# handasontam/PERT-GNN-KDD23

Measured on AMD Instinct MI355X. Metric: training graphs/sec (whole node), higher is better.
Workload: dtype bf16; 1 GPU; model=PERT-GNN 8L/256H, global_batch=1024, vocab=realistic, interfaces=2041, entry_unions=266, graph_mode=full, parallelism=dp1

## Files before the change

csrc/bindings.cpp:

```cpp
#include <hip/hip_runtime.h>
#include <torch/extension.h>

#include <climits>
#include <cstdlib>
#include <memory>
#include <optional>
#include <string>
#include <vector>

#include <c10/cuda/CUDAStream.h>

#include "hip/attn_bn.h"
#include "hip/gemm_dispatch.h"

namespace {

#define CHECK_IN(t)                                                      \
  TORCH_CHECK((t).is_cuda(), #t " must be on GPU");                      \
  TORCH_CHECK((t).is_contiguous(), #t " must be contiguous")

inline hipStream_t cur_stream() {
  return (hipStream_t)c10::cuda::getCurrentCUDAStream().stream();
}

// ... 147 lines not shown
void launch_gemm_f32_nt(const float*, const float*, const float*, float*, int,
                        int, int, bool, hipStream_t);
void launch_gemm_f32_nn(const float*, const float*, const float*, float*, int,
                        int, int, bool, hipStream_t);
void launch_gemm_f32_tn(const float*, const float*, float*, float*, int, int,
                        int, hipStream_t);
void launch_colsum(const float*, float*, long, int, hipStream_t);
void launch_gemm_bf16_nt(const float*, const float*, const float*, float*,
                         int, int, int, bool, hipStream_t);
void launch_gemm_bf16_nn(const float*, const float*, const float*, float*,
                         int, int, int, bool, hipStream_t);
void launch_gemm_bf16_tn(const float*, const float*, float*, float*, int, int,
                         int, hipStream_t);
void launch_gemm_fp16_nt(const float*, const float*, const float*, float*,
                         int, int, int, bool, hipStream_t);
void launch_gemm_fp16_nn(const float*, const float*, const float*, float*,
                         int, int, int, bool, hipStream_t);
void launch_gemm_fp16_tn(const float*, const float*, float*, float*, int, int,
                         int, hipStream_t);
void launch_embed_grouped_scatter(const float*, const int*, const int*, float*,
                                  float*, long, int, int, int, int, int,
                                  hipStream_t);
void launch_embed_grouped_scatter_bal(const void*, int, const int*,
                                      const int*, const int*, const int*,
                                      const int*, const int*, float*, float*,
                                      float*, int, int, int, int, int, int,
                                      hipStream_t);
void launch_rows_sum_lists(const void*, int, const int*, const int*, void*, int,
                           int, int, int, hipStream_t);
void launch_rows_sum_lists_wide(const void*, int, int, const int*, const int*,
                                float*, int, int, int, int, int, hipStream_t);
void launch_embed_fold_gemm(const float*, const float*, float*, int, int, int,
                            int, int, bool, hipStream_t);
void launch_vocab_scatter(const float*, const long*, long, float*, long, int,
                          int, int, int, hipStream_t);
void launch_vocab_scatter_dual(const float*, const long*, int, float*, float*,
                               long, int, int, int, hipStream_t);
void launch_edge_attn_fused_fwd(const float*, const float*, const float*,
                                const long*, int, const int*, const int*,
                                float*, float*, int, int, int, hipStream_t);
void launch_edge_attn_fused_bwd(const float*, const float*, const float*,
                                const float*, const long*, int, const float*,
                                const int*, const int*, const int*,
                                const int*, const int*, float*, float*,
                                float*, int, int, long, int, hipStream_t);
void launch_edge_attn_fused_fwd16(const void*, const void*, const void*,
                                  int, const long*, int, const int*,
                                  const int*, void*, int, float*, int, int,
                                  int, hipStream_t);
void launch_edge_attn_fused_bwd16(const void*, int, const void*,
                                  const void*, const void*, int, const long*,
                                  int, const float*, const int*, const int*,
                                  const int*, const int*, const int*, void*,
                                  void*, float*, int, int, long, int,
                                  hipStream_t, const AttnBnBwd* = nullptr,
                                  const AttnPoolBwd* = nullptr);
void launch_bn_bwd_partials_affine16(const void*, const void*,
                                     const unsigned char*, const float*,
                                     const float*, long, int, float*, float,
                                     float*, float*, float*, hipStream_t,
                                     bool acc = false);
void launch_edge_attn_fused_infer(const float*, const float*, const float*,
                                  const long*, int, const int*, const int*,
                                  const float*, const float*, int, float*,
                                  int, int, int, hipStream_t);
void launch_edge_attn_fused_infer16(const void*, const void*, const void*,
                                    int, const long*, int, const int*,
                                    const int*, const float*, const float*,
                                    int, void*, int, int, int, int,
                                    hipStream_t);
void launch_vocab_scatter_dual16(const void*, const long*, int, float*,
                                 float*, long, int, int, int, hipStream_t);
void launch_gemm_bf16_nt_o16(const float*, const float*, const float*, void*,
                             int, int, int, hipStream_t);
void launch_gemm_a16_glds_nt(const void*, const void*, const float*, void*,
                             int, int, int, int, bool, hipStream_t);
void launch_convert_w16(const float*, void*, long, hipStream_t);
void launch_convert_w16_both(const float*, void*, void*, int, int,
                             hipStream_t);
void launch_gemm_a16_glds_tn(const void*, const void*, float*, float*, int,
                             int, int, hipStream_t, bool acc = false,
                             int tile = 0);
int glds_tn_tile_for(int m, int n, int k2, int tile);
void set_glds_tn_tile(int tile);
void launch_transpose_convert_w16(const float*, void*, int, int, hipStream_t);
void launch_gemm_skinny_nn(const void*, const float*, float*, int, int, int,
                           hipStream_t);
void launch_gemm_bf16_nn_a16(const void*, const float*, float*, int, int, int,
                             hipStream_t);
void launch_gemm_bf16_tn_a16(const void*, const float*, float*, float*, int,
                             int, int, hipStream_t, bool acc = false);
int ptables_max_groups();
void launch_ptables_fwd(int, const float* const*, const float* const*,
                        void* const*, const int*, int, int, hipStream_t);
void launch_ptables_dgrad(const void* const*, const float* const*, const int*,
                          float* const*, const int*, int, int, const bool*,
                          hipStream_t);
bool launch_ptables_wgrad(int, const void* const*, const float* const*,
                          float* const*, const int*, int, bool, hipStream_t,
                          const bool* sink = nullptr);
std::vector<torch::Tensor> collate_native(
    std::vector<torch::Tensor>, std::vector<torch::Tensor>,
    std::vector<torch::Tensor>, std::vector<torch::Tensor>,
    std::vector<torch::Tensor>, std::vector<torch::Tensor>,
    std::vector<torch::Tensor>, std::vector<torch::Tensor>,
    std::vector<torch::Tensor>, bool);


std::vector<torch::Tensor> edge_attn_fwd(torch::Tensor q, torch::Tensor k,
                                         torch::Tensor v, torch::Tensor e,
                                         torch::Tensor row_ptr,
                                         torch::Tensor csr_src,
                                         torch::Tensor skip) {
  CHECK_IN(q); CHECK_IN(k); CHECK_IN(v); CHECK_IN(e);
  CHECK_IN(row_ptr); CHECK_IN(csr_src);
  const int n = q.size(0);
  const int h = q.size(1);
  TORCH_CHECK(h <= 512, "H must be <= 512");
  auto out = torch::empty_like(q);
  auto alpha = torch::empty({e.size(0)}, q.options());
  const float* skip_p = nullptr;
  if (skip.defined() && skip.numel() > 0) {
    CHECK_IN(skip);
    skip_p = skip.data_ptr<float>();
  }
  launch_edge_attn_fwd(q.data_ptr<float>(), k.data_ptr<float>(),
                       v.data_ptr<float>(), e.data_ptr<float>(),
                       row_ptr.data_ptr<int>(), csr_src.data_ptr<int>(),
                       skip_p, out.data_ptr<float>(), alpha.data_ptr<float>(),
                       n, h, cur_stream());
  return {out, alpha};
}

std::vector<torch::Tensor> edge_attn_bwd(
    torch::Tensor g, torch::Tensor q, torch::Tensor k, torch::Tensor v,
    torch::Tensor e, torch::Tensor alpha, torch::Tensor row_ptr,
    torch::Tensor csr_src, torch::Tensor col_ptr, torch::Tensor csc_dst,
    torch::Tensor csc_eid) {
  CHECK_IN(g); CHECK_IN(q); CHECK_IN(alpha);
  const int n = q.size(0);
  const int h = q.size(1);
  const long ne = e.size(0);
  auto dq = torch::empty_like(q);
  auto dk = torch::empty_like(k);
  auto dv = torch::empty_like(v);
  auto de = torch::empty_like(e);
  auto dek = torch::empty_like(e);
  auto dev = torch::empty_like(e);
  launch_edge_attn_bwd(g.data_ptr<float>(), q.data_ptr<float>(),
                       k.data_ptr<float>(), v.data_ptr<float>(),
                       e.data_ptr<float>(), alpha.data_ptr<float>(),
                       row_ptr.data_ptr<int>(), csr_src.data_ptr<int>(),
                       col_ptr.data_ptr<int>(), csc_eid.data_ptr<int>(),
                       dq.data_ptr<float>(), dk.data_ptr<float>(),
                       dv.data_ptr<float>(), de.data_ptr<float>(),
                       dek.data_ptr<float>(), dev.data_ptr<float>(), n, h, ne,
                       cur_stream());
  return {dq, dk, dv, de};
}

torch::Tensor seg_pool_fwd(torch::Tensor x, torch::Tensor probs,
                           torch::Tensor nn, torch::Tensor batch_ptr,
                           int64_t num_graphs) {
  CHECK_IN(x); CHECK_IN(probs); CHECK_IN(nn); CHECK_IN(batch_ptr);
  const int h = x.size(1);
  const long n = x.size(0);
// ... 1185 lines not shown
    torch::Tensor csc_dst, torch::Tensor csc_eid, int64_t heads = 1) {
  CHECK_IN(gout); CHECK_IN(probs); CHECK_IN(nn); CHECK_IN(batch);
  CHECK_IN(qkvs); CHECK_IN(alpha);
  const int n = qkvs.size(0);
  const int h = qkvs.size(1) / 4;
  const long ne = ea.size(0);
  TORCH_CHECK(h == 256 || h == 512, "edge_attn_pool_bwd16 covers H = 256, 512");
  TORCH_CHECK(qkvs.scalar_type() == torch::kBFloat16,
              "edge_attn_pool_bwd16 takes bf16 qkvs");
  TORCH_CHECK(gout.scalar_type() == torch::kFloat32 && gout.dim() == 2 &&
                  gout.size(1) == h,
              "gout must be fp32 [graphs, h]");
  TORCH_CHECK(probs.scalar_type() == torch::kFloat32 &&
                  nn.scalar_type() == torch::kFloat32 &&
                  batch.scalar_type() == torch::kInt64 &&
                  probs.numel() == n && nn.numel() == n && batch.numel() == n,
              "probs/nn (fp32) and batch (int64) must have one entry per node");
  TORCH_CHECK(heads >= 1 && heads <= h && h % heads == 0,
              "heads must divide H (H=", h, ", heads=", heads, ")");
  TORCH_CHECK(alpha.scalar_type() == torch::kFloat32 &&
                  alpha.numel() == ne * heads,
              "alpha must be the fp32 [E, heads] tensor of the forward");
  TORCH_CHECK(pifc.scalar_type() == prpc.scalar_type(),
              "P tables must share a dtype");
  AttnPoolBwd pool{};
  pool.gout = gout.data_ptr<float>();
  pool.probs = probs.data_ptr<float>();
  pool.nn = nn.data_ptr<float>();
  pool.batch = batch.data_ptr<long>();
  auto fopt = qkvs.options().dtype(torch::kFloat32);
  auto dqkvs = torch::empty_like(qkvs);
  auto de = torch::empty({ne, h}, qkvs.options());
  auto dal = torch::empty({ne * heads}, fopt);
  const int p16 = pifc.scalar_type() == torch::kBFloat16 ? 1 : 0;
  launch_edge_attn_fused_bwd16(
      nullptr, 0, qkvs.data_ptr(), pifc.data_ptr(), prpc.data_ptr(), p16,
      ea.data_ptr<long>(), (int)ea.size(1), alpha.data_ptr<float>(),
      row_ptr.data_ptr<int>(), csr_src.data_ptr<int>(),
      col_ptr.data_ptr<int>(), csc_dst.data_ptr<int>(),
      csc_eid.data_ptr<int>(), dqkvs.data_ptr(), de.data_ptr(),
      dal.data_ptr<float>(), n, h, ne, (int)heads, cur_stream(), nullptr,
      &pool);
  return {dqkvs, de};
}

torch::Tensor seg_pool_fwd16(torch::Tensor x, torch::Tensor probs,
                             torch::Tensor nn, torch::Tensor batch_ptr,
                             int64_t num_graphs) {
  CHECK_IN(x); CHECK_IN(probs); CHECK_IN(nn); CHECK_IN(batch_ptr);
  const int h = x.size(1);
  const long n = x.size(0);
  long p = 8192 / std::max<int64_t>(num_graphs, 1);
  const long per_g = (n + std::max<int64_t>(num_graphs, 1) - 1) /
                     std::max<int64_t>(num_graphs, 1);
  p = std::min<long>(std::max<long>(std::min(p, per_g), 1), 64);
  auto fopt = x.options().dtype(torch::kFloat32);
  auto partial = torch::empty({num_graphs * p, h}, fopt);
  auto out = torch::empty({num_graphs, h}, fopt);
  launch_seg_pool_fwd16(x.data_ptr(), probs.data_ptr<float>(),
                        nn.data_ptr<float>(), batch_ptr.data_ptr<int>(),
                        partial.data_ptr<float>(), out.data_ptr<float>(),
                        (int)num_graphs, (int)p, h, cur_stream());
  return out;
}

torch::Tensor seg_pool_bwd16(torch::Tensor gout, torch::Tensor probs,
                             torch::Tensor nn, torch::Tensor batch) {
  CHECK_IN(gout); CHECK_IN(batch);
  const long n = batch.size(0);
  const int h = gout.size(1);
  auto dx = torch::empty({n, h}, gout.options().dtype(torch::kBFloat16));
  launch_seg_pool_bwd16(gout.data_ptr<float>(), probs.data_ptr<float>(),
                        nn.data_ptr<float>(), batch.data_ptr<long>(),
                        dx.data_ptr(), n, h, cur_stream());
  return dx;
}

using gemm_dispatch::dgrad_glds_ok;

static std::vector<torch::Tensor> linear_fwd_a16o16_impl(torch::Tensor x,
                                                         torch::Tensor w,
                                                         torch::Tensor b,
                                                         bool fp16c,
                                                         bool want_wt) {
  CHECK_IN(x); CHECK_IN(w);
  const int m = x.size(0);
  const int k = x.size(1);
  const int n = w.size(0);
  auto y = torch::empty({m, n}, x.options());
  auto wt16 = torch::empty({0}, x.options());
  if (m == 0) return {y, wt16};
  const float* bias = nullptr;
  if (b.defined() && b.numel() > 0) bias = b.data_ptr<float>();
  if (fp16c) {
    launch_gemm_fp16_nt_a16o16(x.data_ptr(), w.data_ptr<float>(), bias,
                               y.data_ptr(), m, n, k, cur_stream());
    return {y, wt16};
  }
  if (gemm_dispatch::fwd_glds_ok(m, n, k)) {
    auto w16 = torch::empty({n, k}, x.options());
    if (want_wt && dgrad_glds_ok(m, n, k)) {
      wt16 = torch::empty({k, n}, x.options());
      launch_convert_w16_both(w.data_ptr<float>(), w16.data_ptr(),
                              wt16.data_ptr(), n, k, cur_stream());
    } else {
      launch_convert_w16(w.data_ptr<float>(), w16.data_ptr(), (long)n * k,
                         cur_stream());
    }
    launch_gemm_a16_glds_nt(x.data_ptr(), w16.data_ptr(), bias, y.data_ptr(),
                            1, m, n, k, false, cur_stream());
    return {y, wt16};
  }
  launch_gemm_bf16_nt_a16o16(x.data_ptr(), w.data_ptr<float>(), bias,
                             y.data_ptr(), m, n, k, cur_stream());
  return {y, wt16};
}

std::vector<torch::Tensor> convert_w16_both(torch::Tensor w) {
  CHECK_IN(w);
  TORCH_CHECK(w.scalar_type() == torch::kFloat32 && w.dim() == 2,
              "w must be fp32 [n, k]");
  const int n = w.size(0);
  const int k = w.size(1);
  auto opt = w.options().dtype(torch::kBFloat16);
  auto w16 = torch::empty({n, k}, opt);
  auto wt16 = torch::empty({k, n}, opt);
  launch_convert_w16_both(w.data_ptr<float>(), w16.data_ptr(),
                          wt16.data_ptr(), n, k, cur_stream());
  return {w16, wt16};
}

torch::Tensor linear_fwd_a16o16(torch::Tensor x, torch::Tensor w,
                                torch::Tensor b, bool fp16c = false) {
  return linear_fwd_a16o16_impl(x, w, b, fp16c, false)[0];
}

std::vector<torch::Tensor> linear_fwd_a16o16_wt(torch::Tensor x,
                                                torch::Tensor w,
                                                torch::Tensor b,
                                                bool fp16c = false) {
  return linear_fwd_a16o16_impl(x, w, b, fp16c, true);
}

torch::Tensor linear_dgrad16_o16(torch::Tensor g, torch::Tensor w,
                                 bool fp16c = false,
                                 c10::optional<torch::Tensor> wt16_in =
                                     c10::nullopt) {
  CHECK_IN(g); CHECK_IN(w);
  const int m = g.size(0);
  const int n = w.size(0);
  const int k = w.size(1);
  auto dx = torch::empty({m, k}, g.options());
  if (m == 0) return dx;
  if (fp16c) {
    launch_gemm_fp16_nn_a16o16(g.data_ptr(), w.data_ptr<float>(),
                               dx.data_ptr(), m, n, k, cur_stream());
    return dx;
  }
  if (dgrad_glds_ok(m, n, k)) {
    torch::Tensor wt16;
    if (wt16_in.has_value() && wt16_in->defined() && wt16_in->numel() > 0) {
      wt16 = *wt16_in;
      CHECK_IN(wt16);
      TORCH_CHECK(wt16.scalar_type() == torch::kBFloat16 && wt16.dim() == 2 &&
                      wt16.size(0) == k && wt16.size(1) == n,
                  "wt16 must be the bf16 [k, n] image of w");
    } else {
      wt16 = torch::empty({k, n}, g.options());
      launch_transpose_convert_w16(w.data_ptr<float>(), wt16.data_ptr(), n, k,
                                   cur_stream());
    }
    launch_gemm_a16_glds_nt(g.data_ptr(), wt16.data_ptr(), nullptr,
                            dx.data_ptr(), 1, m, k, n, false,
                            cur_stream());
    return dx;
  }
  launch_gemm_bf16_nn_a16o16(g.data_ptr(), w.data_ptr<float>(),
                             dx.data_ptr(), m, n, k, cur_stream());
  return dx;
}

std::vector<torch::Tensor> linear_wgrad16_b16(torch::Tensor g, torch::Tensor x,
                                              bool has_bias,
                                              bool fp16c = false,
                                              OptTensor dw_sink = std::nullopt,
                                              OptTensor db_sink = std::nullopt,
                                              int64_t tile = 0) {
  CHECK_IN(g); CHECK_IN(x);
  const int m = x.size(0);
  const int k = x.size(1);
  const int n = g.size(1);
  const char* det = getenv("PERTGNN_DETERMINISTIC");
  const bool glds = gemm_dispatch::wgrad_glds_ok(m, n, k, det && det[0] == '1');
  TORCH_CHECK(tile == 0 ||
                  (glds && !fp16c && glds_tn_tile_for(m, n, k, (int)tile) > 0),
              "linear_wgrad16_b16: tile ", tile, " cannot run [", m, ", ", n,
              "]^T x [", m, ", ", k, "] (needs bf16 compute, m >= 512, n "
              "and k multiples of the tile, not deterministic)");
  auto fopt = x.options().dtype(torch::kFloat32);
  float* dw_ptr = grad_sink(dw_sink, x, {n, k}, "linear_wgrad16_b16");
  float* db_ptr = grad_sink(db_sink, x, {n}, "linear_wgrad16_b16");
  const bool acc = dw_ptr != nullptr;
  TORCH_CHECK((db_ptr != nullptr) == (acc && has_bias),
              "linear_wgrad16_b16: a db sink comes with a dw sink and a bias");
  torch::Tensor dw = torch::empty({0}, fopt), db = torch::empty({0}, fopt);
  if (m == 0) {
    if (acc) return {dw, db};
    return {torch::zeros({n, k}, fopt), torch::zeros({has_bias ? n : 0}, fopt)};
  }
  if (!acc) {
    const long nk = (long)n * k;
    auto buf = torch::empty({nk + (has_bias ? n : 0)}, fopt);
    dw = buf.narrow(0, 0, nk).view({n, k});
    dw_ptr = dw.data_ptr<float>();
    if (has_bias) {
      db = buf.narrow(0, nk, n);
      db_ptr = db.data_ptr<float>();
    }
  }
  if (fp16c) {
    launch_gemm_fp16_tn_a16b16(g.data_ptr(), x.data_ptr(), dw_ptr, db_ptr, m,
                               n, k, cur_stream(), acc);
    return {dw, db};
  }
  if (glds) {
    launch_gemm_a16_glds_tn(g.data_ptr(), x.data_ptr(), dw_ptr, db_ptr, m, n,
                            k, cur_stream(), acc, (int)tile);
    return {dw, db};
  }
  launch_gemm_bf16_tn_a16b16(g.data_ptr(), x.data_ptr(), dw_ptr, db_ptr, m, n,
                             k, cur_stream(), acc);
  return {dw, db};
}

std::string linear_path(const std::string& op, int64_t m64, int64_t n64,
                        int64_t k64, const std::string& io, int64_t prec,
                        bool deterministic) {
  namespace gd = gemm_dispatch;
  TORCH_CHECK(m64 >= 0 && n64 > 0 && k64 > 0 && m64 <= INT_MAX &&
                  n64 <= INT_MAX && k64 <= INT_MAX,
              "linear_path: bad shape");
  const int m = (int)m64, n = (int)n64, k = (int)k64;
  const int iop = op == "fwd" ? 0 : op == "dgrad" ? 1 : op == "wgrad" ? 2 : -1;
  TORCH_CHECK(iop >= 0, "linear_path: op must be fwd, dgrad or wgrad");
  const bool f32io = io == "f32", o16 = io == "o16", a16 = io == "a16";
  TORCH_CHECK(f32io || o16 || a16, "linear_path: io must be f32, o16 or a16");
  TORCH_CHECK(f32io ? (prec >= 0 && prec <= 2)
                    : o16 ? prec == 1 : (prec == 1 || prec == 2),
              "linear_path: no binding with this io and prec");
  if (m == 0) return "none";
  const std::string fp16 = prec == 2 ? "_fp16" : "";
  const std::string fam = prec == 0 ? "f32" : "reg";
  const auto tile = [](bool big) { return big ? "128" : "64"; };
  if (iop == 0) {
    if (a16 && prec == 1 && gd::fwd_glds_ok(m, n, k))
      return gd::glds_nt_wide(m, n, k) ? "glds_nt_128x256" : "glds_nt_128x128";
    return fam + "_nt_" + tile(gd::tile128(m, n)) + fp16;
  }
  if (iop == 1) {
    if (a16 && prec == 1 && gd::dgrad_glds_ok(m, n, k))
      return gd::glds_nt_wide(m, k, n) ? "glds_nt_128x256" : "glds_nt_128x128";
    if (o16 && gd::dgrad_skinny(m)) return "skinny_nn";
    return fam + "_nn_" + tile(gd::tile128(m, k)) + fp16;
  }
  if (a16 && prec == 1 && gd::wgrad_glds_ok(m, n, k, deterministic))
    return "glds_tn/s=" +
           std::to_string(gd::glds_tn_slices(
               m, gd::glds_tn_tiles(gd::glds_tn_tile(m, n, k), n, k)));
  return fam + "_tn_" + tile(gd::tn_tile128(n, k)) + fp16 + "/s=" +
         std::to_string(gd::tn_slices(m, gd::tn_tiles(n, k),
                                      prec == 0 ? 32 : 64, deterministic));
}

std::string wgrad_tile(int64_t m, int64_t n, int64_t k, bool deterministic) {
  TORCH_CHECK(m >= 0 && n > 0 && k > 0 && m <= INT_MAX && n <= INT_MAX &&
                  k <= INT_MAX, "wgrad_tile: bad shape");
  if (!gemm_dispatch::wgrad_glds_ok((int)m, (int)n, (int)k, deterministic))
    return "none";
  return gemm_dispatch::tn_tile_name(
      glds_tn_tile_for((int)m, (int)n, (int)k, gemm_dispatch::TN_AUTO));
}

void set_wgrad_tile(int64_t tile) {
  TORCH_CHECK(tile >= 0 && tile <= gemm_dispatch::TN_256x256,
              "set_wgrad_tile: tile must be 0 (auto), 1, 2 or 3");
  set_glds_tn_tile((int)tile);
}

std::vector<std::string> linear_path_labels() {
  std::vector<std::string> out;
  const auto add = [&](const char* io, int prec, const char* op,
                       const std::string& label) {
    out.push_back(std::string(io) + "|" + std::to_string(prec) + "|" + op +
                  "|" + label);
  };
  const auto reg = [&](const char* io, int prec) {
    const std::string fam = prec == 0 ? "f32" : "reg";
    const std::string fp16 = prec == 2 ? "_fp16" : "";
    for (const char* t : {"64", "128"}) {
      add(io, prec, "fwd", fam + "_nt_" + t + fp16);
      add(io, prec, "dgrad", fam + "_nn_" + t + fp16);
      for (const char* s : {"/s=1", "/s>1"})
        add(io, prec, "wgrad", fam + "_tn_" + t + fp16 + s);
    }
  };
  for (int prec = 0; prec <= 2; ++prec) reg("f32", prec);
  reg("o16", 1);
  add("o16", 1, "dgrad", "skinny_nn");
  reg("a16", 1);
  reg("a16", 2);
  for (const char* op : {"fwd", "dgrad"})
    for (const char* l : {"glds_nt_128x128", "glds_nt_128x256"})
      add("a16", 1, op, l);
  for (const char* s : {"/s=1", "/s>1"})
    add("a16", 1, "wgrad", std::string("glds_tn") + s);
  return out;
}


namespace {

int ptables_check(const torch::Tensor& ifc_table,
                  const torch::Tensor& rpc_table,
                  const std::vector<torch::Tensor>& we_ifc,
                  const std::vector<torch::Tensor>& we_rpc) {
  CHECK_IN(ifc_table); CHECK_IN(rpc_table);
  TORCH_CHECK(ifc_table.dim() == 2 && rpc_table.dim() == 2,
              "ptables: tables must be 2-D");
  TORCH_CHECK(ifc_table.scalar_type() == torch::kFloat32 &&
                  rpc_table.scalar_type() == torch::kFloat32,
              "ptables: tables must be float32");
  const int64_t h = ifc_table.size(1);
  TORCH_CHECK(h > 0 && rpc_table.size(1) == h,
              "ptables: tables must share a non-empty hidden size");
  TORCH_CHECK(!we_ifc.empty() && we_ifc.size() == we_rpc.size(),
              "ptables: need one we_ifc and one we_rpc per layer, got ",
              we_ifc.size(), " and ", we_rpc.size());
  for (const auto* list : {&we_ifc, &we_rpc})
    for (const auto& w : *list) {
      TORCH_CHECK(w.is_cuda() && w.device() == ifc_table.device(),
                  "ptables: weight must be on the tables' GPU");
      TORCH_CHECK(w.is_contiguous(), "ptables: weight must be contiguous");
      TORCH_CHECK(w.scalar_type() == torch::kFloat32,
                  "ptables: weight must be float32");
      TORCH_CHECK(w.dim() == 2 && w.size(0) == h && w.size(1) == h,
                  "ptables: weight must be [", h, ", ", h, "]");
    }
  TORCH_CHECK(ifc_table.size(0) < (1 << 30) && rpc_table.size(0) < (1 << 30) &&
                  h < (1 << 15),
              "ptables: table too large");
  return (int)h;
}

}

std::vector<torch::Tensor> ptables_fwd(torch::Tensor ifc_table,
                                       torch::Tensor rpc_table,
                                       std::vector<torch::Tensor> we_ifc,
                                       std::vector<torch::Tensor> we_rpc) {
  const int h = ptables_check(ifc_table, rpc_table, we_ifc, we_rpc);
  const int layers = (int)we_ifc.size();
  auto opt = ifc_table.options().dtype(torch::kBFloat16);
  std::vector<torch::Tensor> out;
  std::vector<const float*> a, w;
  std::vector<void*> c;
  std::vector<int> m;
  for (int t = 0; t < 2; ++t) {
    const auto& table = t == 0 ? ifc_table : rpc_table;
    const auto& ws = t == 0 ? we_ifc : we_rpc;
// ... 164 lines not shown
          py::arg("relu"), py::arg("keep_inv") = 1.0,
          py::arg("dgamma_sink") = py::none(),
          py::arg("dbeta_sink") = py::none());
  mod.def("vocab_scatter", &vocab_scatter);
  mod.def("collate_native", &collate_native,
          py::call_guard<py::gil_scoped_release>());
  mod.def("edge_attn_fused_fwd", &edge_attn_fused_fwd, py::arg("qkvs"),
          py::arg("pifc"), py::arg("prpc"), py::arg("edge_attr"),
          py::arg("row_ptr"), py::arg("csr_src"), py::arg("out16"),
          py::arg("heads") = 1);
  mod.def("edge_attn_fused_bwd", &edge_attn_fused_bwd, py::arg("g"),
          py::arg("qkvs"), py::arg("pifc"), py::arg("prpc"),
          py::arg("edge_attr"), py::arg("alpha"), py::arg("row_ptr"),
          py::arg("csr_src"), py::arg("col_ptr"), py::arg("csc_dst"),
          py::arg("csc_eid"), py::arg("heads") = 1);
  mod.def("edge_attn_fused_infer", &edge_attn_fused_infer, py::arg("qkvs"),
          py::arg("pifc"), py::arg("prpc"), py::arg("edge_attr"),
          py::arg("row_ptr"), py::arg("csr_src"), py::arg("bn_scale"),
          py::arg("bn_shift"), py::arg("relu"), py::arg("out16"),
          py::arg("heads") = 1);
  mod.def("embed_grouped_scatter", &embed_grouped_scatter);
  mod.def("linear_fwd", &linear_fwd);
  mod.def("linear_fwd_bf16", &linear_fwd_bf16);
  mod.def("linear_fwd_fp16", &linear_fwd_fp16);
  mod.def("linear_bwd_fp16", &linear_bwd_fp16);
  mod.def("linear_bwd_bf16", &linear_bwd_bf16);
  mod.def("gemm_nt_bf16", &gemm_nt_bf16);
  mod.def("gemm_nn_bf16", &gemm_nn_bf16);
  mod.def("gemm_tn_bf16", &gemm_tn_bf16);
  mod.def("linear_bwd", &linear_bwd);
  mod.def("gemm_nt", &gemm_nt);
  mod.def("gemm_nn", &gemm_nn);
  mod.def("gemm_tn", &gemm_tn);
  mod.def("edge_attn_fwd", &edge_attn_fwd);
  mod.def("edge_attn_bwd", &edge_attn_bwd);
  mod.def("seg_pool_fwd", &seg_pool_fwd);
  mod.def("seg_pool_bwd", &seg_pool_bwd);
  mod.def("embed_node_fwd", &embed_node_fwd, py::arg("x_raw"), py::arg("idx"), py::arg("table"), py::arg("out16") = false, py::arg("pad_to") = 0);
  mod.def("embed_edge_fwd", &embed_edge_fwd);
  mod.def("gather_rows", &gather_rows);
  mod.def("bn_relu_fwd16", &bn_relu_fwd16, py::arg("x"), py::arg("gamma"),
          py::arg("beta"), py::arg("running_mean"), py::arg("running_var"),
          py::arg("momentum"), py::arg("eps"), py::arg("training"),
          py::arg("relu"), py::arg("dropout_p") = 0.0,
          py::arg("seed") = torch::Tensor());
  mod.def("bn_relu_bwd16", &bn_relu_bwd16, py::arg("g"), py::arg("x"),
          py::arg("gamma"), py::arg("mean"), py::arg("invstd"), py::arg("y"),
          py::arg("relu"), py::arg("keep_inv") = 1.0,
          py::arg("dgamma_sink") = py::none(),
          py::arg("dbeta_sink") = py::none());
  mod.def("bn_finalize_apply16", &bn_finalize_apply16, py::arg("x"),
          py::arg("partials"), py::arg("gamma"), py::arg("beta"),
          py::arg("running_mean"), py::arg("running_var"), py::arg("momentum"),
          py::arg("eps"), py::arg("training"), py::arg("relu"),
          py::arg("dropout_p") = 0.0, py::arg("seed") = torch::Tensor());
  mod.def("bn_bwd_partials16", &bn_bwd_partials16, py::arg("g"), py::arg("x"),
          py::arg("y"), py::arg("mean"), py::arg("invstd"), py::arg("relu"),
          py::arg("keep_inv") = 1.0);
  mod.def("bn_bwd_apply16", &bn_bwd_apply16, py::arg("g"), py::arg("x"),
          py::arg("y"), py::arg("mean"), py::arg("invstd"), py::arg("gamma"),
          py::arg("partials_global"), py::arg("partials_local"),
          py::arg("relu"), py::arg("keep_inv") = 1.0,
          py::arg("dgamma_sink") = py::none(),
          py::arg("dbeta_sink") = py::none());
  mod.def("edge_attn_bn_bwd16", &edge_attn_bn_bwd16, py::arg("g"),
          py::arg("x"), py::arg("mask"), py::arg("gamma"), py::arg("mean"),
          py::arg("invstd"), py::arg("keep_inv"), py::arg("qkvs"),
          py::arg("pifc"), py::arg("prpc"), py::arg("edge_attr"),
          py::arg("alpha"), py::arg("row_ptr"), py::arg("csr_src"),
          py::arg("col_ptr"), py::arg("csc_dst"), py::arg("csc_eid"),
          py::arg("heads") = 1, py::arg("partials_global") = py::none(),
          py::arg("partials_local") = py::none(),
          py::arg("dgamma_sink") = py::none(),
          py::arg("dbeta_sink") = py::none());
  mod.def("edge_attn_pool_bwd16", &edge_attn_pool_bwd16, py::arg("gout"),
          py::arg("probs"), py::arg("nn"), py::arg("batch"), py::arg("qkvs"),
          py::arg("pifc"), py::arg("prpc"), py::arg("edge_attr"),
          py::arg("alpha"), py::arg("row_ptr"), py::arg("csr_src"),
          py::arg("col_ptr"), py::arg("csc_dst"), py::arg("csc_eid"),
          py::arg("heads") = 1);
  mod.def("seg_pool_fwd16", &seg_pool_fwd16);
  mod.def("seg_pool_bwd16", &seg_pool_bwd16);
  mod.def("linear_fwd_a16o16", &linear_fwd_a16o16, py::arg("x"), py::arg("w"),
          py::arg("b"), py::arg("fp16c") = false);
  mod.def("convert_w16_both", &convert_w16_both, py::arg("w"));
  mod.def("linear_fwd_a16o16_wt", &linear_fwd_a16o16_wt, py::arg("x"),
          py::arg("w"), py::arg("b"), py::arg("fp16c") = false);
  mod.def("linear_dgrad16_o16", &linear_dgrad16_o16, py::arg("g"),
          py::arg("w"), py::arg("fp16c") = false,
          py::arg("wt16") = py::none());
  mod.def("linear_wgrad16_b16", &linear_wgrad16_b16, py::arg("g"),
          py::arg("x"), py::arg("has_bias"), py::arg("fp16c") = false,
          py::arg("dw_sink") = py::none(), py::arg("db_sink") = py::none(),
          py::arg("tile") = 0);
  mod.def("wgrad_tile", &wgrad_tile, py::arg("m"), py::arg("n"), py::arg("k"),
          py::arg("deterministic") = false);
  mod.def("set_wgrad_tile", &set_wgrad_tile, py::arg("tile"));
  mod.def("linear_path", &linear_path, py::arg("op"), py::arg("m"),
          py::arg("n"), py::arg("k"), py::arg("io"), py::arg("prec"),
          py::arg("deterministic") = false);
  mod.def("linear_path_labels", &linear_path_labels);
  mod.def("bn_relu_fwd", &bn_relu_fwd, py::arg("x"), py::arg("gamma"),
          py::arg("beta"), py::arg("running_mean"), py::arg("running_var"),
          py::arg("momentum"), py::arg("eps"), py::arg("training"),
          py::arg("relu"), py::arg("dropout_p") = 0.0,
          py::arg("seed") = torch::Tensor());
  mod.def("bn_relu_bwd", &bn_relu_bwd, py::arg("g"), py::arg("x"),
          py::arg("gamma"), py::arg("mean"), py::arg("invstd"), py::arg("y"),
          py::arg("relu"), py::arg("keep_inv") = 1.0,
          py::arg("dgamma_sink") = py::none(),
          py::arg("dbeta_sink") = py::none());
  mod.def("quantile_loss_fwd", &quantile_loss_fwd);
  mod.def("quantile_loss_bwd", &quantile_loss_bwd);
  mod.def("eval_metrics", &eval_metrics);
  mod.def("adam_step_dynamic", &adam_step_dynamic);
  mod.def("adam_step", &adam_step, py::arg("p"), py::arg("g"), py::arg("m"),
          py::arg("v"), py::arg("state"), py::arg("lr"), py::arg("b1"),
          py::arg("b2"), py::arg("eps"), py::arg("gscale") = 1.0);
}
```

csrc/hip/gemm_bf16.hip:

```cpp

#include "common.h"
#include "gemm_dispatch.h"

static inline bool pertgnn_deterministic() {
  const char* e = getenv("PERTGNN_DETERMINISTIC");
  return e && e[0] == '1';
}
#include <cstdlib>

#define BGEMM_PAD 8
#define BGEMM_THREADS 256

typedef __attribute__((ext_vector_type(4))) float f32x4;
typedef __attribute__((ext_vector_type(8))) __bf16 bf16x8;
typedef __attribute__((ext_vector_type(4))) __bf16 bf16x4;
typedef __attribute__((ext_vector_type(8))) _Float16 f16x8;
typedef __attribute__((ext_vector_type(4))) _Float16 f16x4;

template <typename T16> struct Vec16;
template <> struct Vec16<__bf16> {
  using v4 = bf16x4;
  using v8 = bf16x8;
  static __device__ __forceinline__ f32x4 mfma(v8 a, v8 b, f32x4 c) {
    return __builtin_amdgcn_mfma_f32_16x16x32_bf16(a, b, c, 0, 0, 0);
// ... 891 lines not shown
    for (int j = 0; j < FN; ++j) acc[i][j] = {0.f, 0.f, 0.f, 0.f};

  stage.template operator()<GRPS_A>(a, a_base, 0, lds_ab(0));
  stage.template operator()<GRPS_B>(b, b_base, 0, lds_bb(0));
  asm volatile("s_waitcnt vmcnt(0)" ::: "memory");
  __syncthreads();

  const int fi = lane & 15;
  const int fk = (lane >> 4) * 8;
  auto mma = [&](const __bf16* la, const __bf16* lb) {
#pragma unroll
    for (int s = 0; s < BK / 32; ++s) {
      const int kb = (s * 32 + fk) * 2;
      bf16x8 av[FM], bv[FN];
#pragma unroll
      for (int mi = 0; mi < FM; ++mi) {
        const int row = wm + mi * 16 + fi;
        av[mi] = *reinterpret_cast<const bf16x8*>(
            (const char*)la + glds_swz((unsigned)(row * (BK * 2) + kb)));
      }
#pragma unroll
      for (int ni = 0; ni < FN; ++ni) {
        const int row = wn + ni * 16 + fi;
        bv[ni] = *reinterpret_cast<const bf16x8*>(
            (const char*)lb + glds_swz((unsigned)(row * (BK * 2) + kb)));
      }
#pragma unroll
      for (int mi = 0; mi < FM; ++mi)
#pragma unroll
        for (int ni = 0; ni < FN; ++ni)
          acc[mi][ni] = __builtin_amdgcn_mfma_f32_16x16x32_bf16(
              av[mi], bv[ni], acc[mi][ni], 0, 0, 0);
    }
  };

  int buf = 0;
  for (int k0 = BK; k0 < k; k0 += BK) {
    stage.template operator()<GRPS_A>(a, a_base, k0, lds_ab(buf ^ 1));
    stage.template operator()<GRPS_B>(b, b_base, k0, lds_bb(buf ^ 1));
    mma(lds_ab(buf), lds_bb(buf));
    asm volatile("s_waitcnt vmcnt(0)" ::: "memory");
    __syncthreads();
    buf ^= 1;
  }
  mma(lds_ab(buf), lds_bb(buf));

  __syncthreads();
  constexpr int BNW = BN / WCOL;
  constexpr int SW = BNW + 8;
  TO* scratch = reinterpret_cast<TO*>(smem + wave * 16 * SW * sizeof(TO));
  const int fcol = lane & 15;
  const int frow = (lane >> 4) * 4;
  constexpr int EPL = 16 / sizeof(TO);
  constexpr int CPR = BNW / EPL;
#pragma unroll
  for (int mi = 0; mi < FM; ++mi) {
#pragma unroll
    for (int ni = 0; ni < FN; ++ni)
#pragma unroll
      for (int r = 0; r < 4; ++r) {
        const int col = ni * 16 + fcol;
        float v = acc[mi][ni][r];
        if (bias) v += bias[n0 + wn + col];
        if (relu) v = fmaxf(v, 0.f);
        scratch[(frow + r) * SW + col] = (TO)v;
      }
    asm volatile("s_waitcnt lgkmcnt(0)" ::: "memory");
#pragma unroll
    for (int it = 0; it < 16 * CPR / PERTGNN_WAVE; ++it) {
      const int chunk = it * PERTGNN_WAVE + lane;
      const int r = chunk / CPR;
      const int off = (chunk % CPR) * EPL;
      const u32x4_t val = *reinterpret_cast<const u32x4_t*>(&scratch[r * SW + off]);
      const int grow = m0 + wm + mi * 16 + r;
      if (grow >= m) continue;
      u32x4_t* dst =
          reinterpret_cast<u32x4_t*>(&c[(long)grow * n + n0 + wn + off]);
      if constexpr (NTC)
        __builtin_nontemporal_store(val, dst);
      else
        *dst = val;
    }
    asm volatile("s_waitcnt lgkmcnt(0)" ::: "memory");
  }
}

__global__ void convert_w16_kernel(const float* __restrict__ w,
                                   __bf16* __restrict__ o, long numel) {
  const long i0 = (long)blockIdx.x * blockDim.x + threadIdx.x;
  const long stride = (long)gridDim.x * blockDim.x;
  for (long t = i0; t < numel; t += stride) o[t] = (__bf16)w[t];
}

__global__ void transpose_convert_w16_kernel(const float* __restrict__ w,
                                             __bf16* __restrict__ o, int rows,
                                             int cols) {
  __shared__ float tile[32][33];
  const int c0 = blockIdx.x * 32;
  const int r0 = blockIdx.y * 32;
  const int tx = threadIdx.x % 32;
  const int ty = threadIdx.x / 32;
  for (int dy = ty; dy < 32; dy += blockDim.x / 32) {
    const int r = r0 + dy, ccol = c0 + tx;
    tile[dy][tx] = (r < rows && ccol < cols) ? w[(long)r * cols + ccol] : 0.f;
  }
  __syncthreads();
  for (int dy = ty; dy < 32; dy += blockDim.x / 32) {
    const int ccol = c0 + dy, r = r0 + tx;
    if (ccol < cols && r < rows) o[(long)ccol * rows + r] = (__bf16)tile[tx][dy];
  }
}

__global__ void convert_w16_both_kernel(const float* __restrict__ w,
                                        __bf16* __restrict__ o,
                                        __bf16* __restrict__ ot, int rows,
                                        int cols) {
  __shared__ float tile[32][33];
  const int c0 = blockIdx.x * 32;
  const int r0 = blockIdx.y * 32;
  const int tx = threadIdx.x % 32;
  const int ty = threadIdx.x / 32;
  for (int dy = ty; dy < 32; dy += blockDim.x / 32) {
    const int r = r0 + dy, ccol = c0 + tx;
    float v = 0.f;
    if (r < rows && ccol < cols) {
      v = w[(long)r * cols + ccol];
      o[(long)r * cols + ccol] = (__bf16)v;
    }
    tile[dy][tx] = v;
  }
  __syncthreads();
  for (int dy = ty; dy < 32; dy += blockDim.x / 32) {
    const int ccol = c0 + dy, r = r0 + tx;
    if (ccol < cols && r < rows)
      ot[(long)ccol * rows + r] = (__bf16)tile[tx][dy];
  }
}

void launch_convert_w16_both(const float* w, void* o, void* ot, int rows,
                             int cols, hipStream_t s) {
  convert_w16_both_kernel<<<dim3((cols + 31) / 32, (rows + 31) / 32),
                            dim3(256), 0, s>>>(w, (__bf16*)o, (__bf16*)ot,
                                               rows, cols);
}

void launch_convert_w16(const float* w, void* o, long numel, hipStream_t s) {
  const int blocks = (int)min((numel + 255) / 256, (long)4096);
  convert_w16_kernel<<<blocks, 256, 0, s>>>(w, (__bf16*)o, numel);
}

void launch_transpose_convert_w16(const float* w, void* o, int rows, int cols,
                                  hipStream_t s) {
  transpose_convert_w16_kernel<<<dim3((cols + 31) / 32, (rows + 31) / 32),
                                 dim3(256), 0, s>>>(w, (__bf16*)o, rows, cols);
}

static int glds_bk() {
  static int v = [] {
    const char* e = getenv("PERTGNN_GLDS_BK");
    return (e && atoi(e) == 64) ? 64 : 32;
  }();
  return v;
}
static bool glds_t512() {
  static bool v = [] {
    const char* e = getenv("PERTGNN_GLDS_T512");
    return !(e && atoi(e) == 0);
  }();
  return v;
}
static bool glds_ntc() {
  static bool v = [] {
    const char* e = getenv("PERTGNN_GLDS_NTC");
    return !(e && atoi(e) == 0);
  }();
  return v;
}


static bool glds_n256() {
  static bool v = [] {
    const char* e = getenv("PERTGNN_GLDS_N256");
    return !(e && atoi(e) == 0);
  }();
  return v;
}

void launch_gemm_a16_glds_nt(const void* a_v, const void* b16_v,
                             const float* bias, void* c_v, int c16, int m,
                             int n, int k, bool relu, hipStream_t s) {
  const __bf16* a = (const __bf16*)a_v;
  const __bf16* b = (const __bf16*)b16_v;
  constexpr int BM = 128, BN = 128;
  if (m <= 0) return;
  const int mt = (m + BM - 1) / BM;
  if (gemm_dispatch::glds_nt_wide(m, n, k) && glds_n256()) {
    if (c16)
      gemm_a16_glds_nt_kernel<128, 256, 32, __bf16, 512, true>
          <<<dim3(mt), dim3(512), 0, s>>>(a, b, bias, (__bf16*)c_v, m, n, k,
                                          relu ? 1 : 0);
    else
      gemm_a16_glds_nt_kernel<128, 256, 32, float, 512, true>
          <<<dim3(mt), dim3(512), 0, s>>>(a, b, bias, (float*)c_v, m, n, k,
                                          relu ? 1 : 0);
  } else {
    const int grid = mt * (n / BN);
    const int bk = glds_bk();
    const bool t512 = glds_t512();
    const bool ntc = glds_ntc();
#define GLDS_DISPATCH(BKV, TH, NTCV)                                           \
  do {                                                                         \
    if (c16)                                                                   \
      gemm_a16_glds_nt_kernel<BM, BN, BKV, __bf16, TH, NTCV>                   \
          <<<dim3(grid), dim3(TH), 0, s>>>(a, b, bias, (__bf16*)c_v, m, n, k,  \
                                           relu ? 1 : 0);                      \
    else                                                                       \
      gemm_a16_glds_nt_kernel<BM, BN, BKV, float, TH, NTCV>                    \
          <<<dim3(grid), dim3(TH), 0, s>>>(a, b, bias, (float*)c_v, m, n, k,   \
                                           relu ? 1 : 0);                      \
  } while (0)
    if ((bk == 32 || k % 64 != 0) && k % 32 == 0) {
      if (t512) { if (ntc) GLDS_DISPATCH(32, 512, true); else GLDS_DISPATCH(32, 512, false); }
      else      { if (ntc) GLDS_DISPATCH(32, 256, true); else GLDS_DISPATCH(32, 256, false); }
    } else {
      if (t512) { if (ntc) GLDS_DISPATCH(64, 512, true); else GLDS_DISPATCH(64, 512, false); }
      else      { if (ntc) GLDS_DISPATCH(64, 256, true); else GLDS_DISPATCH(64, 256, false); }
    }
#undef GLDS_DISPATCH
  }
}


typedef __attribute__((ext_vector_type(4))) __bf16 bf16x4_g;

template <int BM , int BN , int BKM ,
          int THREADS = 512, bool ACC = false>
__launch_bounds__(THREADS)
__global__ void gemm_a16_glds_tn_kernel(const __bf16* __restrict__ a,
                                        const __bf16* __restrict__ b,
                                        float* __restrict__ c,
                                        float* __restrict__ dbias, int m,
                                        int n, int k2, int slices) {
  constexpr int NWAVE = THREADS / PERTGNN_WAVE;
  constexpr int WCOL = NWAVE / 2;
  constexpr int FM = (BM / 2) / 16, FN = (BN / WCOL) / 16;
  constexpr int OCTS = BKM / 8;
  constexpr int GROUP_BYTES = OCTS * 1024;
  constexpr int TILE_BYTES = BM * BKM * 2;
  constexpr int GRPS_A = TILE_BYTES / 1024 / NWAVE;
  constexpr int GRPS_B = BN * BKM * 2 / 1024 / NWAVE;
  static_assert(GRPS_A * NWAVE * 1024 == TILE_BYTES &&
                    GRPS_B * NWAVE * 1024 == BN * BKM * 2,
                "every wave stages whole 1-KiB groups of both images");
  __shared__ char smem[2 * (BM + BN) * BKM * 2];
  const auto lds_ab = [&](int i) { return smem + i * TILE_BYTES; };
  const auto lds_bb = [&](int i) {
    return smem + 2 * TILE_BYTES + i * (BN * BKM * 2);
  };
  const int bid = xcd_swizzle(blockIdx.x, gridDim.x);
  const int tiles_k = k2 / BN;
  const int tile_id = bid / slices;
  const int slice = bid % slices;
  const int n0 = (tile_id / tiles_k) * BM;
  const int k0 = (tile_id % tiles_k) * BN;
  const int wave = threadIdx.x / PERTGNN_WAVE;
  const int lane = threadIdx.x % PERTGNN_WAVE;
  const int wm = (wave / WCOL) * (BM / 2);
  const int wn = (wave % WCOL) * (BN / WCOL);

  const int m_full = m - m % BKM;
  const int per_slice = ((m_full / BKM + slices - 1) / slices) * BKM;
  const int c_beg = slice * per_slice;
  const int c_end = min(m_full, c_beg + per_slice);
  if (c_beg >= c_end) return;

  auto stage = [&]<int GRPS_PER_WAVE, bool TAIL = false>(
                   const __bf16* src_base, long ld, int col0, int mrow0,
                   char* lds) {
#pragma unroll
    for (int i = 0; i < GRPS_PER_WAVE; ++i) {
      const int grp = wave + i * NWAVE;
      int mrow = mrow0 + (grp % OCTS) * 8 + ((lane >> 1) & 7);
      if constexpr (TAIL) mrow = min(mrow, m - 1);
      const int col = (grp / OCTS) * 64 + (lane >> 4) * 16 + (lane & 1) * 8;
      const __bf16* src = src_base + (long)mrow * ld + col0 + col;
      __builtin_amdgcn_global_load_lds(
          (const __attribute__((address_space(1))) void*)src,
          (__attribute__((address_space(3))) void*)(lds + grp * 1024),
          16, 0, 0);
    }
  };

  f32x4 acc[FM][FN];
  float dbacc[FM];
#pragma unroll
  for (int i = 0; i < FM; ++i) {
    dbacc[i] = 0.f;
#pragma unroll
    for (int j = 0; j < FN; ++j) acc[i][j] = {0.f, 0.f, 0.f, 0.f};
  }

  stage.template operator()<GRPS_A>(a, n, n0, c_beg, lds_ab(0));
  stage.template operator()<GRPS_B>(b, k2, k0, c_beg, lds_bb(0));
  asm volatile("s_waitcnt vmcnt(0)" ::: "memory");
  __syncthreads();

  const bool do_bias = (dbias != nullptr) && (k0 == 0) && wave % WCOL == 0;

  auto frag = [&](const char* img, int block16, int s) {
    const char* p = img + (block16 >> 2) * GROUP_BYTES +
                    (s * 4 + (lane >> 4)) * 1024 + (block16 & 3) * 256 +
                    (lane & 15) * 8;
    bf16x4_g lo = __builtin_amdgcn_ds_read_tr16_b64_v4bf16(
        (__attribute__((address_space(3))) bf16x4_g*)p);
// ... 542 lines not shown
```

csrc/hip/gemm_dispatch.h:

```cpp
#pragma once

namespace gemm_dispatch {

inline bool tile128(int m, int cols) { return m >= 512 && cols >= 128; }

inline bool tn_tile128(int n, int k2) { return n >= 128 && k2 >= 128; }

inline int tn_tiles(int n, int k2) {
  const int b = tn_tile128(n, k2) ? 128 : 64;
  return ((n + b - 1) / b) * ((k2 + b - 1) / b);
}

inline int tn_slices(int m, int tiles, int step, bool deterministic) {
  int slices = 1;
  while (!deterministic && tiles * slices < 512 && slices < 64 &&
         (long)slices * step * 4 < m)
    slices *= 2;
  return slices;
}

inline bool fwd_glds_ok(int m, int n, int k) {
  return m >= 512 && n % 128 == 0 && k % 32 == 0;
}

inline bool dgrad_glds_ok(int m, int n, int k) {
  return m >= 512 && k % 128 == 0 && n % 64 == 0;
}

inline bool wgrad_glds_ok(int m, int n, int k, bool deterministic) {
  return !deterministic && m >= 512 && n % 128 == 0 && k % 128 == 0;
}

inline bool glds_nt_wide(int m, int cols, int contract) {
  return m / 128 >= 1024 && cols == 256 && contract % 32 == 0;
}

inline int glds_tn_slices(int m, int tiles) {
  constexpr int BKM = 64;
  int slices = 1;
  while (tiles * slices < 512 && slices < 64 &&
         (long)slices * BKM * 4 < m - m % BKM)
    slices *= 2;
  return slices;
}

enum TnTile { TN_AUTO = 0, TN_128x128 = 1, TN_256x128 = 2, TN_256x256 = 3 };

inline int tn_tile_rows(int tile) { return tile == TN_128x128 ? 128 : 256; }
inline int tn_tile_cols(int tile) { return tile == TN_256x256 ? 256 : 128; }
inline const char* tn_tile_name(int tile) {
  return tile == TN_256x256 ? "256x256"
         : tile == TN_256x128 ? "256x128" : "128x128";
}

inline bool glds_tn_tile_ok(int tile, int m, int n, int k) {
  return tile >= TN_128x128 && tile <= TN_256x256 && m >= 512 &&
         n % tn_tile_rows(tile) == 0 && k % tn_tile_cols(tile) == 0;
}

inline int glds_tn_tile(int , int , int ) { return TN_128x128; }

inline int glds_tn_tiles(int tile, int n, int k) {
  return (n / tn_tile_rows(tile)) * (k / tn_tile_cols(tile));
}

inline bool dgrad_skinny(int m) { return m <= 16; }

}
```

Measured before the change: 129,300 graphs/s.

## Add A-resident forward GEMM kernel for k=256 large-m linear layers

Adds a forward NT GEMM kernel that loads the whole A row-block (k=256) into LDS once, then sweeps all N tiles while double-buffering B slabs via global_load_lds. It is selected automatically when m is large (at least 57344), k is 256, n is a multiple of 128, and the existing wide-stream path does not apply. The aim is to avoid re-reading activations for every N tile and to cut per-tile prologue cost. The trade-off is heavy LDS use per block, which limits occupancy, and more B traffic per block. Also adds an optional output buffer argument and variant overrides.

Result: faster. 132,000 graphs/s (median of 6 runs) (+2.1%).

```diff
diff --git a/csrc/bindings.cpp b/csrc/bindings.cpp
--- a/csrc/bindings.cpp
+++ b/csrc/bindings.cpp
@@ -253,6 +253,10 @@
                              int, int, hipStream_t, bool acc = false,
                              int tile = 0);
 int glds_tn_tile_for(int m, int n, int k2, int tile);
+void launch_gemm_a16_resident_nt(const void*, const void*, const float*, void*,
+                                 int, int, int, hipStream_t);
+int fwd_variant_for(int m, int n, int k);
+void set_fwd_variant_hook(int v);
 void set_glds_tn_tile(int tile);
 void launch_transpose_convert_w16(const float*, void*, int, int, hipStream_t);
 void launch_gemm_skinny_nn(const void*, const float*, float*, int, int, int,
@@ -1604,12 +1608,34 @@
                                                          torch::Tensor w,
                                                          torch::Tensor b,
                                                          bool fp16c,
-                                                         bool want_wt) {
+                                                         bool want_wt,
+                                                         int64_t variant = 0,
+                                                         OptTensor out =
+                                                             std::nullopt) {
+  namespace gd = gemm_dispatch;
   CHECK_IN(x); CHECK_IN(w);
   const int m = x.size(0);
   const int k = x.size(1);
   const int n = w.size(0);
-  auto y = torch::empty({m, n}, x.options());
+  TORCH_CHECK(variant == gd::FWD_AUTO ||
+                  (!fp16c && variant == gd::FWD_STREAM &&
+                   gd::fwd_stream_can(m, n, k)) ||
+                  (!fp16c && variant == gd::FWD_RESIDENT &&
+                   gd::fwd_resident_can(m, n, k)),
+              "linear_fwd_a16o16: variant ", variant, " cannot run [", m, ", ",
+              k, "] x [", n, ", ", k, "]^T (1 needs bf16 compute, n % 128 == "
+              "0 and k % 32 == 0; 2 needs bf16 compute, n % 128 == 0 and k == "
+              "256)");
+  torch::Tensor y;
+  if (out.has_value() && out->defined()) {
+    CHECK_IN((*out));
+    TORCH_CHECK(out->scalar_type() == torch::kBFloat16 && out->dim() == 2 &&
+                    out->size(0) >= m && out->size(1) == n,
+                "out must be bf16 [>= m, n]");
+    y = out->narrow(0, 0, m);
+  } else {
+    y = torch::empty({m, n}, x.options());
+  }
   auto wt16 = torch::empty({0}, x.options());
   if (m == 0) return {y, wt16};
   const float* bias = nullptr;
@@ -1619,7 +1645,9 @@
                                y.data_ptr(), m, n, k, cur_stream());
     return {y, wt16};
   }
-  if (gemm_dispatch::fwd_glds_ok(m, n, k)) {
+  const int fv = variant != gd::FWD_AUTO ? (int)variant
+                                         : fwd_variant_for(m, n, k);
+  if (fv != 0) {
     auto w16 = torch::empty({n, k}, x.options());
     if (want_wt && dgrad_glds_ok(m, n, k)) {
       wt16 = torch::empty({k, n}, x.options());
@@ -1629,8 +1657,13 @@
       launch_convert_w16(w.data_ptr<float>(), w16.data_ptr(), (long)n * k,
                          cur_stream());
     }
-    launch_gemm_a16_glds_nt(x.data_ptr(), w16.data_ptr(), bias, y.data_ptr(),
-                            1, m, n, k, false, cur_stream());
+    if (fv == gd::FWD_RESIDENT)
+      launch_gemm_a16_resident_nt(x.data_ptr(), w16.data_ptr(), bias,
+                                  y.data_ptr(), m, n, k, cur_stream());
+    else
+      launch_gemm_a16_glds_nt(x.data_ptr(), w16.data_ptr(), bias,
+                              y.data_ptr(), 1, m, n, k, false,
+                              cur_stream());
     return {y, wt16};
   }
   launch_gemm_bf16_nt_a16o16(x.data_ptr(), w.data_ptr<float>(), bias,
@@ -1653,8 +1686,10 @@
 }
 
 torch::Tensor linear_fwd_a16o16(torch::Tensor x, torch::Tensor w,
-                                torch::Tensor b, bool fp16c = false) {
-  return linear_fwd_a16o16_impl(x, w, b, fp16c, false)[0];
+                                torch::Tensor b, bool fp16c = false,
+                                int64_t variant = 0,
+                                OptTensor out = std::nullopt) {
+  return linear_fwd_a16o16_impl(x, w, b, fp16c, false, variant, out)[0];
 }
 
 std::vector<torch::Tensor> linear_fwd_a16o16_wt(torch::Tensor x,
@@ -1807,6 +1842,21 @@
   TORCH_CHECK(tile >= 0 && tile <= gemm_dispatch::TN_256x256,
               "set_wgrad_tile: tile must be 0 (auto), 1, 2 or 3");
   set_glds_tn_tile((int)tile);
+}
+
+std::string fwd_variant(int64_t m, int64_t n, int64_t k) {
+  TORCH_CHECK(m >= 0 && n > 0 && k > 0 && m <= INT_MAX && n <= INT_MAX &&
+                  k <= INT_MAX, "fwd_variant: bad shape");
+  const int v = m == 0 ? 0 : fwd_variant_for((int)m, (int)n, (int)k);
+  return v == gemm_dispatch::FWD_RESIDENT ? "resident"
+         : v == gemm_dispatch::FWD_STREAM ? "stream" : "none";
+}
+
+void set_fwd_variant(int64_t variant) {
+  TORCH_CHECK(variant >= 0 && variant <= gemm_dispatch::FWD_RESIDENT,
+              "set_fwd_variant: variant must be 0 (auto), 1 (stream) or 2 "
+              "(resident)");
+  set_fwd_variant_hook((int)variant);
 }
 
 std::vector<std::string> linear_path_labels() {
@@ -2137,7 +2187,11 @@
   mod.def("seg_pool_fwd16", &seg_pool_fwd16);
   mod.def("seg_pool_bwd16", &seg_pool_bwd16);
   mod.def("linear_fwd_a16o16", &linear_fwd_a16o16, py::arg("x"), py::arg("w"),
-          py::arg("b"), py::arg("fp16c") = false);
+          py::arg("b"), py::arg("fp16c") = false, py::arg("variant") = 0,
+          py::arg("out") = py::none());
+  mod.def("fwd_variant", &fwd_variant, py::arg("m"), py::arg("n"),
+          py::arg("k"));
+  mod.def("set_fwd_variant", &set_fwd_variant, py::arg("variant"));
   mod.def("convert_w16_both", &convert_w16_both, py::arg("w"));
   mod.def("linear_fwd_a16o16_wt", &linear_fwd_a16o16_wt, py::arg("x"),
           py::arg("w"), py::arg("b"), py::arg("fp16c") = false);
diff --git a/csrc/hip/gemm_bf16.hip b/csrc/hip/gemm_bf16.hip
--- a/csrc/hip/gemm_bf16.hip
+++ b/csrc/hip/gemm_bf16.hip
@@ -997,6 +997,156 @@
         *dst = val;
     }
     asm volatile("s_waitcnt lgkmcnt(0)" ::: "memory");
+  }
+}
+
+template <int BM, int KT, int BKB, bool NTC>
+__launch_bounds__(BM * 4)
+__global__ void gemm_a16_resident_nt_kernel(const __bf16* __restrict__ a,
+                                            const __bf16* __restrict__ b,
+                                            const float* __restrict__ bias,
+                                            __bf16* __restrict__ c, int m,
+                                            int n) {
+  constexpr int BN = 128;
+  constexpr int THREADS = BM * 4;
+  constexpr int NWAVE = THREADS / PERTGNN_WAVE;
+  constexpr int FM = 2, FN = 4;
+  constexpr int SLAB_A = BM * 64;
+  constexpr int SLAB_B = BN * 64;
+  constexpr int NSLAB = BKB / 32;
+  constexpr int KS = KT / BKB;
+  constexpr int A_BYTES = (KT / 32) * SLAB_A;
+  constexpr int B_BYTES = NSLAB * SLAB_B;
+  constexpr int GRPS_B = B_BYTES / 1024;
+  constexpr int BNW = 64;
+  constexpr int SW = BNW + 8;
+  static_assert(SLAB_A / 1024 == NWAVE, "one glds per wave per A slab");
+  static_assert(KS % 2 == 0 && GRPS_B % NWAVE == 0, "ring of two stages");
+  __shared__ char smem[A_BYTES + 2 * B_BYTES + NWAVE * 16 * SW * 2];
+  char* const lds_a = smem;
+  const auto lds_bb = [&](int i) { return smem + A_BYTES + i * B_BYTES; };
+  const int m0 = blockIdx.x * BM;
+  const int wave = threadIdx.x / PERTGNN_WAVE;
+  const int lane = threadIdx.x % PERTGNN_WAVE;
+  const int wm = (wave / 2) * 32;
+  const int wn = (wave % 2) * BNW;
+
+  const unsigned l_off = glds_swz((unsigned)lane * 16);
+  const int src_row = (int)(l_off / 64);
+  const int src_kb = (int)(l_off % 64);
+  const long ldb = (long)KT * 2;
+
+  const auto glds16 = [](const char* src, char* dst) {
+    __builtin_amdgcn_global_load_lds(
+        (const __attribute__((address_space(1))) void*)src,
+        (__attribute__((address_space(3))) void*)dst, 16, 0, 0);
+  };
+  const auto stage_b = [&](int n0, int ks, char* lds) {
+#pragma unroll
+    for (int i = 0; i < GRPS_B / NWAVE; ++i) {
+      const int grp = wave + i * NWAVE;
+      const int row = n0 + (grp % 8) * 16 + src_row;
+      const int kb = (ks * BKB + (grp / 8) * 32) * 2 + src_kb;
+      glds16((const char*)b + (long)row * ldb + kb, lds + grp * 1024);
+    }
+  };
+
+  {
+    const int row = min(m0 + wave * 16 + src_row, m - 1);
+    const char* src = (const char*)a + (long)row * ldb + src_kb;
+#pragma unroll
+    for (int s = 0; s < KT / 32; ++s)
+      glds16(src + s * 64, lds_a + s * SLAB_A + wave * 1024);
+  }
+  stage_b(0, 0, lds_bb(0));
+  asm volatile("s_waitcnt vmcnt(0)" ::: "memory");
+  __syncthreads();
+
+  const int fi = lane & 15;
+  const int kb = (lane >> 4) * 16;
+  const int fcol = lane & 15;
+  const int frow = (lane >> 4) * 4;
+  __bf16* scratch = reinterpret_cast<__bf16*>(smem + A_BYTES + 2 * B_BYTES +
+                                              wave * 16 * SW * 2);
+  const int tiles_n = n / BN;
+  for (int ct = 0; ct < tiles_n; ++ct) {
+    const int n0 = ct * BN;
+    f32x4 acc[FM][FN];
+#pragma unroll
+    for (int i = 0; i < FM; ++i)
+#pragma unroll
+      for (int j = 0; j < FN; ++j) acc[i][j] = {0.f, 0.f, 0.f, 0.f};
+
+#pragma unroll
+    for (int ks = 0; ks < KS; ++ks) {
+      if (ks + 1 < KS)
+        stage_b(n0, ks + 1, lds_bb((ks + 1) & 1));
+      else if (ct + 1 < tiles_n)
+        stage_b(n0 + BN, 0, lds_bb(0));
+      const char* lb = lds_bb(ks & 1);
+#pragma unroll
+      for (int s = 0; s < NSLAB; ++s) {
+        const char* la = lds_a + (ks * NSLAB + s) * SLAB_A;
+        bf16x8 av[FM], bv[FN];
+#pragma unroll
+        for (int mi = 0; mi < FM; ++mi) {
+          const int row = wm + mi * 16 + fi;
+          av[mi] = *reinterpret_cast<const bf16x8*>(
+              la + glds_swz((unsigned)(row * 64 + kb)));
+        }
+#pragma unroll
+        for (int ni = 0; ni < FN; ++ni) {
+          const int row = wn + ni * 16 + fi;
+          bv[ni] = *reinterpret_cast<const bf16x8*>(
+              lb + s * SLAB_B + glds_swz((unsigned)(row * 64 + kb)));
+        }
+#pragma unroll
+        for (int mi = 0; mi < FM; ++mi)
+#pragma unroll
+          for (int ni = 0; ni < FN; ++ni)
+            acc[mi][ni] = __builtin_amdgcn_mfma_f32_16x16x32_bf16(
+                av[mi], bv[ni], acc[mi][ni], 0, 0, 0);
+      }
+      asm volatile("s_waitcnt vmcnt(0)" ::: "memory");
+      __syncthreads();
+    }
+
+    float bv4[FN] = {0.f, 0.f, 0.f, 0.f};
+    if (bias) {
+#pragma unroll
+      for (int ni = 0; ni < FN; ++ni)
+        bv4[ni] = bias[n0 + wn + ni * 16 + fcol];
+    }
+    constexpr int CPR = BNW / 8;
+#pragma unroll
+    for (int mi = 0; mi < FM; ++mi) {
+#pragma unroll
+      for (int ni = 0; ni < FN; ++ni)
+#pragma unroll
+        for (int r = 0; r < 4; ++r) {
+          float v = acc[mi][ni][r];
+          if (bias) v += bv4[ni];
+          scratch[(frow + r) * SW + ni * 16 + fcol] = (__bf16)v;
+        }
+      asm volatile("s_waitcnt lgkmcnt(0)" ::: "memory");
+#pragma unroll
+      for (int it = 0; it < 16 * CPR / PERTGNN_WAVE; ++it) {
+        const int chunk = it * PERTGNN_WAVE + lane;
+        const int r = chunk / CPR;
+        const int off = (chunk % CPR) * 8;
+        const u32x4_t val =
+            *reinterpret_cast<const u32x4_t*>(&scratch[r * SW + off]);
+        const int grow = m0 + wm + mi * 16 + r;
+        if (grow >= m) continue;
+        u32x4_t* dst =
+            reinterpret_cast<u32x4_t*>(&c[(long)grow * n + n0 + wn + off]);
+        if constexpr (NTC)
+          __builtin_nontemporal_store(val, dst);
+        else
+          *dst = val;
+      }
+      asm volatile("s_waitcnt lgkmcnt(0)" ::: "memory");
+    }
   }
 }
 
@@ -1145,6 +1295,39 @@
   }
 }
 
+static int g_fwd_variant = gemm_dispatch::FWD_AUTO;
+void set_fwd_variant_hook(int v) { g_fwd_variant = v; }
+
+int fwd_variant_for(int m, int n, int k) {
+  const char* e = getenv("PERTGNN_NO_FWD_RESIDENT");
+  return gemm_dispatch::fwd_variant(m, n, k, g_fwd_variant,
+                                    e && e[0] == '1');
+}
+
+static int fwd_resident_geom() {
+  const char* e = getenv("PERTGNN_FWD_RES_GEOM");
+  const int g = e ? atoi(e) : 0;
+  return (g == 1 || g == 2) ? g : gemm_dispatch::FWD_RESIDENT_GEOM;
+}
+
+void launch_gemm_a16_resident_nt(const void* a_v, const void* b16_v,
+                                 const float* bias, void* c_v, int m, int n,
+                                 int k, hipStream_t s) {
+  if (m <= 0) return;
+  const __bf16* a = (const __bf16*)a_v;
+  const __bf16* b = (const __bf16*)b16_v;
+  __bf16* c = (__bf16*)c_v;
+  if (!gemm_dispatch::fwd_resident_can(m, n, k))
+    pertgnn_shape_fail("launch_gemm_a16_resident_nt", k != 256 ? "k" : "n",
+                       k != 256 ? k : n);
+  if (fwd_resident_geom() == 1)
+    gemm_a16_resident_nt_kernel<128, 256, 128, true>
+        <<<dim3((m + 127) / 128), dim3(512), 0, s>>>(a, b, bias, c, m, n);
+  else
+    gemm_a16_resident_nt_kernel<64, 256, 64, true>
+        <<<dim3((m + 63) / 64), dim3(256), 0, s>>>(a, b, bias, c, m, n);
+}
+
 
 typedef __attribute__((ext_vector_type(4))) __bf16 bf16x4_g;
 
diff --git a/csrc/hip/gemm_dispatch.h b/csrc/hip/gemm_dispatch.h
--- a/csrc/hip/gemm_dispatch.h
+++ b/csrc/hip/gemm_dispatch.h
@@ -35,6 +35,29 @@
   return m / 128 >= 1024 && cols == 256 && contract % 32 == 0;
 }
 
+enum FwdVariant { FWD_AUTO = 0, FWD_STREAM = 1, FWD_RESIDENT = 2 };
+
+inline bool fwd_stream_can(int m, int n, int k) {
+  return m >= 1 && n % 128 == 0 && k % 32 == 0;
+}
+inline bool fwd_resident_can(int m, int n, int k) {
+  return m >= 1 && n % 128 == 0 && k == 256;
+}
+
+constexpr int FWD_RESIDENT_GEOM = 1;
+constexpr int FWD_RESIDENT_MIN_M = 57344;
+
+inline bool fwd_resident_ok(int m, int n, int k) {
+  return fwd_glds_ok(m, n, k) && fwd_resident_can(m, n, k) &&
+         m >= FWD_RESIDENT_MIN_M && !glds_nt_wide(m, n, k);
+}
+
+inline int fwd_variant(int m, int n, int k, int forced, bool no_resident) {
+  if (forced != FWD_AUTO && fwd_resident_can(m, n, k)) return forced;
+  if (!fwd_glds_ok(m, n, k)) return 0;
+  return fwd_resident_ok(m, n, k) && !no_resident ? FWD_RESIDENT : FWD_STREAM;
+}
+
 inline int glds_tn_slices(int m, int tiles) {
   constexpr int BKM = 64;
   int slices = 1;
```
